# cvYouTian/Dedark-YOLO

Hardware: AMD Instinct MI355X
Metric: training img/s at 640x640 (higher is better)
Workload: dtype bf16

## Files before the change

dedark_yolo_amd/_C.py:

```python
import ctypes as C
import os

_HERE = os.path.dirname(os.path.abspath(__file__))
LIB_PATH = os.path.join(os.environ.get("DY_LIB_DIR") or os.path.join(_HERE, "lib"), "libdedark_yolo.so")

DY_F32, DY_BF16, DY_F16 = 0, 1, 2
ACT_NONE, ACT_SILU, ACT_LEAKY = 0, 1, 2
OPT_RULES = dict(Adam=0, Adamax=1, NAdam=2, RAdam=3, RMSProp=4)
STATS_REPLICAS = 64
BN_BWD_REPLICAS = 8

vp, i32, i64, f32, f64 = C.c_void_p, C.c_int, C.c_int64, C.c_float, C.c_double


class ConvDesc(C.Structure):
    _fields_ = [("src", vp), ("src_ld", i64), ("N", i32), ("Hs", i32), ("Ws", i32), ("Cs", i32), ("w", vp), ("dst", vp),
                ("dst_ld", i64), ("Hd", i32), ("Wd", i32), ("Cd", i32), ("KH", i32), ("KW", i32), ("stride", i32),
                ("pad", i32), ("dil", i32), ("scale", vp), ("shift", vp), ("act", i32), ("stats", vp), ("accumulate", i32),
                ("dtype", i32), ("dst_row_stride", i64), ("dst_img_stride", i64), ("KHf", i32), ("KWf", i32), ("kh0", i32),
                ("kh_step", i32), ("kw0", i32), ("kw_step", i32), ("dst_valid_channels", i32), ("dst_planar", vp),
                ("add_src", vp), ("add_src_ld", i64)]


class PackItem(C.Structure):
    _fields_ = [("w", vp), ("packed", vp), ("Cout", i32), ("Cout_pad", i32), ("Cin", i32), ("Cin_pad", i32), ("KH", i32),
                ("KW", i32), ("transposed", i32), ("dtype", i32), ("first_block", i64)]


class DetMaps(C.Structure):
    _fields_ = [("map", vp * 3), ("map_ld", i64 * 3), ("h", i32 * 3), ("w", i32 * 3), ("stride", f32 * 3), ("B", i32),
                ("nc", i32), ("n_levels", i32), ("dtype", i32)]


class DetMaps4(DetMaps):
    _fields_ = [("map3", vp), ("map_ld3", i64), ("h3", i32), ("w3", i32), ("stride3", f32)]


class AugSample(C.Structure):
    _fields_ = [("src", vp * 4), ("sh", i32 * 4), ("sw", i32 * 4), ("pitch", i64 * 4), ("rect", (i32 * 6) * 4), ("n_src", i32),
                ("canvas_h", i32), ("canvas_w", i32), ("hsv", i32), ("flipud", i32), ("fliplr", i32), ("minv", C.c_double * 6),
                ("lut", (C.c_uint8 * 256) * 3)]


class AugMixSample(C.Structure):
    _fields_ = [("a", AugSample), ("b", AugSample), ("r", C.c_double), ("r1", C.c_double), ("mix", i32)]


class SegDesc(C.Structure):
    _fields_ = [("mc", vp), ("mc_ld", i64), ("proto", vp), ("proto_ld", i64), ("B", i32), ("A", i32), ("nm", i32), ("mh", i32),
                ("mw", i32), ("target_gt_idx", vp), ("fg_mask", vp), ("target_box", vp), ("masks", vp), ("mask_dtype", i32),
                ("mask_h", i32), ("mask_w", i32), ("overlap", i32), ("gt_rows", vp), ("n_max", i32), ("img_h", f32), ("img_w", f32),
                ("pos", vp), ("npos", vp), ("dtype", i32)]


BIAS_GRAD_CHUNKS = 2048
LN_MAX_C = 2048
LN_MAX_PARTS = 512

POSE_MAX_LEVELS = 4


class PoseDesc(C.Structure):
    _fields_ = [("kpt", vp * POSE_MAX_LEVELS), ("kpt_ld", i64 * POSE_MAX_LEVELS), ("h", i32 * POSE_MAX_LEVELS), ("w", i32 * POSE_MAX_LEVELS),
                ("stride", f32 * POSE_MAX_LEVELS), ("n_levels", i32), ("B", i32), ("A", i32), ("K", i32), ("ndim", i32), ("dtype", i32),
                ("target_gt_idx", vp), ("fg_mask", vp), ("target_box", vp), ("keypoints", vp), ("n_targets", i32), ("gt_rows", vp),
                ("n_max", i32), ("img_h", f32), ("img_w", f32), ("sigma", vp), ("pos", vp), ("npos", vp)]


_SIGS = {
    "dy_version": [],
    "dy_frontend_init": [],
    "dy_conv2d_fwd": [C.POINTER(ConvDesc), vp],
    "dy_conv2d_dgrad": [C.POINTER(ConvDesc), vp],
    "dy_conv2d_wgrad": [vp, i64, i32, i32, i32, i32, vp, i64, i32, i32, i32, i32, i32, i32, i32, i32, i32, i32, vp, i64, vp,
                        i32, vp],
    "dy_conv2d_wgrad_forked": [vp, vp, i64, i32, i32, i32, i32, vp, i64, i32, i32, i32, i32, i32, i32, i32, i32, i32, i32, vp, i64,
                               vp, i32, vp],
    "dy_conv2d_bn_act_fwd": [C.POINTER(ConvDesc), i64, vp, vp, vp, vp, f32, f32, vp, i32, vp, i64, vp, i64, vp],
    "dy_bn_act_bwd": [vp, i64, vp, i64, vp, vp, i32, vp, vp, i64, vp, vp, i64, i32, i32, vp],
# ... 182 lines not shown
```

dedark_yolo_amd/csrc/conv.hip:

```cpp
#include <stdlib.h>
#include "dy_host.h"
#include "conv_epilogue.h"
#include "../../include/dedark_yolo.h"
#include "conv_route.h"

namespace {

constexpr int ROWB = 144;
constexpr int NTHREADS = 256;

struct ConvP {
  const char* src;
  long src_ld;
  int N, Hs, Ws, Cs;
  const char* w;
  char* dst;
  long dst_ld;
  int Hd, Wd, Cd;
  int KH, KW, stride, pad, dil;
  const float* scale;
  const float* shift;
  int act;
  double* stats;
  int accumulate;
// ... 637 lines not shown

template <typename T>
__global__ void pack_weight_kernel(const float* __restrict__ w, T* __restrict__ out, int Cout, int Cout_pad, int Cin,
                                   int Cin_pad, int KH, int KW, int transposed) {
  long total = (long)Cout_pad * KH * KW * Cin_pad;
  for (long i = blockIdx.x * (long)blockDim.x + threadIdx.x; i < total; i += (long)gridDim.x * blockDim.x) {
    int co, kh, kw, ci;
    long r = i;
    if (!transposed) {
      ci = (int)(r % Cin_pad); r /= Cin_pad;
      kw = (int)(r % KW); r /= KW;
      kh = (int)(r % KH); r /= KH;
      co = (int)r;
    } else {
      co = (int)(r % Cout_pad); r /= Cout_pad;
      kw = (int)(r % KW); r /= KW;
      kh = (int)(r % KH); r /= KH;
      ci = (int)r;
    }
    float v = (ci < Cin && co < Cout) ? w[(((long)co * Cin + ci) * KH + kh) * KW + kw] : 0.f;
    DT<T>::st(out + i, v);
  }
}

constexpr int PACK_TILE = 32, PACK_TAPS = 9;

__device__ inline void pack_store(const dy_pack_item& it, long o, float v) {
  if (it.dtype == DY_F32) ((float*)it.packed)[o] = v;
  else if (it.dtype == DY_F16) ((f16_t*)it.packed)[o] = (f16_t)v;
  else ((bf16_t*)it.packed)[o] = f32_to_bf16(v);
}

template <int TC>
__device__ inline void pack_chunk(const dy_pack_item& it, float (&tile)[PACK_TILE][PACK_TILE * PACK_TAPS + 1], int co0, int ci0, int T,
                                  int t0, int tc_rt) {
  const int tc = TC ? TC : tc_rt;
  const int tid = threadIdx.x;
  const int run = PACK_TILE * tc;
  {
    const int r = tid >> 3, co = co0 + r;
    const bool row_ok = co < it.Cout;
    const float* src = it.w + ((long)co * it.Cin + ci0) * T + t0;
    for (int k = tid & 7; k < run; k += 8) {
      const int cl = k / tc, t = k - cl * tc;
      const int ci = ci0 + cl;
      float v = 0.f;
      if (row_ok && ci < it.Cin) v = src[(long)cl * T + t];
      tile[r][cl * PACK_TAPS + t] = v;
    }
  }
  __syncthreads();
  const int VE = it.dtype == DY_F32 ? 4 : 8, GP = PACK_TILE / VE;
  const int n_vec = PACK_TILE * GP * tc;
  for (int i = tid; i < n_vec; i += 256) {
    const int g = i % GP, q = i / GP;
    const int a = q / tc, t = q - a * tc;
    float v[8];
    long o;
    bool ok;
    if (!it.transposed) {
      const int co = co0 + a, ci = ci0 + g * VE;
#pragma unroll
      for (int e = 0; e < 8; ++e) v[e] = e < VE ? tile[a][(g * VE + e) * PACK_TAPS + t] : 0.f;
      ok = co < it.Cout_pad && ci < it.Cin_pad;
      o = ((long)co * T + t0 + t) * it.Cin_pad + ci;
    } else {
      const int ci = ci0 + a, co = co0 + g * VE;
#pragma unroll
      for (int e = 0; e < 8; ++e) v[e] = e < VE ? tile[g * VE + e][a * PACK_TAPS + t] : 0.f;
      ok = co < it.Cout_pad && ci < it.Cin_pad;
      o = ((long)ci * T + t0 + t) * it.Cout_pad + co;
    }
    if (!ok) continue;
    if (it.dtype == DY_F32) stvec<float>((float*)it.packed + o, v);
    else if (it.dtype == DY_F16) stvec<f16_t>((f16_t*)it.packed + o, v);
    else stvec<bf16_t>((bf16_t*)it.packed + o, v);
  }
  __syncthreads();
}

__global__ __launch_bounds__(256) void pack_multi_kernel(const dy_pack_item* __restrict__ items, int n_items) {
  __shared__ float tile[PACK_TILE][PACK_TILE * PACK_TAPS + 1];
  __shared__ long fb[1024];
  const long b = blockIdx.x;
  const bool cached = n_items <= 1024;
  if (cached) {
    for (int i = threadIdx.x; i < n_items; i += 256) fb[i] = items[i].first_block;
    __syncthreads();
  }
  int lo = 0, hi = n_items - 1;
  while (lo < hi) {
    const int mid = (lo + hi + 1) >> 1;
    if ((cached ? fb[mid] : items[mid].first_block) <= b) lo = mid; else hi = mid - 1;
  }
  const dy_pack_item it = items[lo];
  const int tiles_ci = (it.Cin_pad + PACK_TILE - 1) / PACK_TILE;
  const int tb = (int)(b - it.first_block);
  const int co0 = (tb / tiles_ci) * PACK_TILE, ci0 = (tb % tiles_ci) * PACK_TILE;
  const int T = it.KH * it.KW;
  if (T == 9) pack_chunk<9>(it, tile, co0, ci0, 9, 0, 9);
  else if (T == 1) pack_chunk<1>(it, tile, co0, ci0, 1, 0, 1);
  else
    for (int t0 = 0; t0 < T; t0 += PACK_TAPS) pack_chunk<0>(it, tile, co0, ci0, T, t0, T - t0 < PACK_TAPS ? T - t0 : PACK_TAPS);
}

template <typename T, int MODE>
int launch_conv(const dy_conv_desc* d, hipStream_t st, const dy_conv_desc* classes, int ncls) {
  ConvP p;
  dy_route::fill_parity_classes(p, classes, ncls);
  dy_route::fill_gather(p, d);
  constexpr int BM = 128;
  const int tiles_m = dy_cdiv(p.M, BM);
  auto blocks = [&](int bn) {
    p.tiles_n = dy_cdiv(d->Cd, bn);
    p.nblk = tiles_m * p.tiles_n;
    if (p.ncls > 1) p.nblk = dy_route::number_parity_blocks(p, BM, dy_route::CLS_SEQUENTIAL);
  };
  dy_note_kernel(d->Cd <= 32 ? "conv_igemm_kernel<BN=32>" : (d->Cd <= 64 ? "conv_igemm_kernel<BN=64>" : "conv_igemm_kernel<BN=128>"));
  if (d->Cd <= 32) {
    blocks(32);
    conv_igemm_kernel<T, BM, 32, 4, 1, MODE><<<p.nblk, NTHREADS, 0, st>>>(p);
  } else if (d->Cd <= 64) {
    blocks(64);
    conv_igemm_kernel<T, BM, 64, 2, 2, MODE><<<p.nblk, NTHREADS, 0, st>>>(p);
  } else {
    blocks(128);
    conv_igemm_kernel<T, BM, 128, 2, 2, MODE><<<p.nblk, NTHREADS, 0, st>>>(p);
  }
  DY_LAUNCH_CHECK();
// ... 326 lines not shown
```

dedark_yolo_amd/csrc/conv_epilogue.h:

```cpp
#pragma once
#include "dy_common.h"

namespace dy_epi {

template <int BM>
constexpr int pitch() { return BM * 2 + 8; }

typedef __attribute__((ext_vector_type(4))) short s16x4;
typedef __attribute__((address_space(3))) s16x4* lds_s16x4_ptr;

template <int BM, int BN>
constexpr int image_bytes() { return BN * pitch<BM>(); }

template <typename T16 = bf16_t>
__device__ inline uint32_t pack2(float a, float b) {
  if constexpr (__is_same(T16, bf16_t)) return pack_bf16x2(a, b);
  else return (uint32_t)cvt16<T16>(a) | ((uint32_t)cvt16<T16>(b) << 16);
}

template <int BM, int BN, int NW, typename T16, typename OffFn>
__device__ inline void store_image(const char* smem, int lane, int wave, long m0, int n0, long M, int Cd, int accumulate, T16* dst,
                                   OffFn off) {
  constexpr int PT = pitch<BM>();
  constexpr int UP = BM / 16, UC = BN / 32;
  const int g = lane >> 4, li = lane & 15, tq = li >> 2, tp = li & 3;
  static_assert(UP % NW == 0, "pixel tiles per wave");
#pragma unroll 2
  for (int u = 0; u < (UP / NW) * UC; ++u) {
    const int pt = wave + NW * (u / UC), ct = u % UC;
    const int cb = ct * 32 + 8 * g;
    const char* base = smem + (cb + tq) * PT + (pt * 16 + 4 * tp) * 2;
    const s16x4 lo = __builtin_amdgcn_ds_read_tr16_b64_v4i16((lds_s16x4_ptr)(base));
    const s16x4 hi = __builtin_amdgcn_ds_read_tr16_b64_v4i16((lds_s16x4_ptr)(base + 4 * PT));
    const long m = m0 + pt * 16 + li;
    const int n = n0 + cb;
    if (m < M && n < Cd) {
      u32x4 v;
      v[0] = (uint32_t)(uint16_t)lo[0] | ((uint32_t)(uint16_t)lo[1] << 16);
      v[1] = (uint32_t)(uint16_t)lo[2] | ((uint32_t)(uint16_t)lo[3] << 16);
      v[2] = (uint32_t)(uint16_t)hi[0] | ((uint32_t)(uint16_t)hi[1] << 16);
      v[3] = (uint32_t)(uint16_t)hi[2] | ((uint32_t)(uint16_t)hi[3] << 16);
      T16* o = dst + off(m) + n;
      if (n + 8 <= Cd) {
        if (accumulate) {
          float x[8], y[8];
          ldvec<T16>(o, x);
          ldvec<T16>(reinterpret_cast<const T16*>(&v), y);
#pragma unroll
          for (int e = 0; e < 8; ++e) x[e] += y[e];
          stvec<T16>(o, x);
        } else {
          *reinterpret_cast<u32x4*>(o) = v;
        }
      } else {
        const T16* e = reinterpret_cast<const T16*>(&v);
        for (int q = 0; q < 8 && n + q < Cd; ++q) {
          if (accumulate) DT<T16>::st(o + q, DT<T16>::ld(o + q) + DT<T16>::ld(e + q));
          else o[q] = e[q];
        }
      }
    }
  }
}

template <int BN>
constexpr int row_pitch() { return BN * 2 + 8; }

template <int BM, int BN>
constexpr int row_image_bytes() { return BM * row_pitch<BN>(); }

template <int BM, int BN, int NW, typename T16, typename OffFn, int RG = 64>
__device__ inline void store_rows(const char* smem, int lane, int wave, long m0, int n0, long M, int Cd, int accumulate, T16* dst, OffFn off,
                                  const T16* __restrict__ add = nullptr, long add_ld = 0) {
  constexpr int PT = row_pitch<BN>();
  constexpr int LPP = BN >= 128 ? 16 : BN / 8;
  constexpr int PPI = 64 / LPP;
  constexpr int ITERS = BM / PPI / NW;
  constexpr int HALVES = BN >= 128 ? BN / 128 : 1;
  const int pl = lane / LPP, chunk = lane % LPP;
  const bool nt = accumulate & 2;
  accumulate &= 1;
#pragma unroll 2
  for (int u = 0; u < ITERS; ++u) {
    const int px = PPI * (wave + NW * u) + pl;
    if (RG < 64 && (px & 63) >= RG) continue;
    const long m = RG < 64 ? m0 + (px >> 6) * RG + (px & 63) : m0 + px;
#pragma unroll
    for (int h = 0; h < HALVES; ++h) {
      const int c = 128 * h + 8 * chunk;
      const uint2 lo = *reinterpret_cast<const uint2*>(smem + px * PT + c * 2);
      const uint2 hi = *reinterpret_cast<const uint2*>(smem + px * PT + c * 2 + 8);
      const int n = n0 + c;
      if (m < M && n < Cd) {
        u32x4 v = {lo.x, lo.y, hi.x, hi.y};
        T16* o = dst + off(m) + n;
        if (n + 8 <= Cd) {
          if (accumulate || add) {
            float x[8], y[8];
            ldvec<T16>(reinterpret_cast<const T16*>(&v), y);
            if (accumulate) {
              ldvec<T16>(o, x);
#pragma unroll
              for (int e = 0; e < 8; ++e) y[e] += x[e];
            }
            if (add) {
              ldvec<T16>(add + m * add_ld + n, x);
#pragma unroll
              for (int e = 0; e < 8; ++e) y[e] += x[e];
            }
            if (nt) {
              u32x4 w;
              stvec<T16>(reinterpret_cast<T16*>(&w), y);
              asm volatile("global_store_dwordx4 %0, %1, off nt" ::"v"(o), "v"(w) : "memory");
            } else {
              stvec<T16>(o, y);
            }
          } else if (nt) {
            asm volatile("global_store_dwordx4 %0, %1, off nt" ::"v"(o), "v"(v) : "memory");
          } else {
            *reinterpret_cast<u32x4*>(o) = v;
          }
        } else {
          const T16* e = reinterpret_cast<const T16*>(&v);
          for (int q = 0; q < 8 && n + q < Cd; ++q) {
            float t = DT<T16>::ld(e + q);
            if (accumulate) t += DT<T16>::ld(o + q);
            if (add) t += DT<T16>::ld(add + m * add_ld + n + q);
            DT<T16>::st(o + q, t);
          }
        }
      }
    }
  }
}
// ... 48 lines not shown
```

dedark_yolo_amd/csrc/conv_v4.hip:

```cpp
#include <stdlib.h>
#include <type_traits>
#include "dy_host.h"
#include "conv_epilogue.h"
#include "../../include/dedark_yolo.h"
#include "conv_route.h"

namespace v4 {

constexpr int BM = 256, BN = 256, BK = 64;
constexpr int HALF = 128 * 128;
constexpr int OFF_A0 = 0, OFF_A1 = HALF, OFF_B0 = 2 * HALF, OFF_B1 = 3 * HALF, BUF = 4 * HALF;
constexpr unsigned B_ROW_OOB = 0x40000000u;

typedef __attribute__((address_space(3))) void* lds_ptr_t;
typedef __attribute__((ext_vector_type(8))) __bf16 bf16x8;

struct P {
  const char* src;
  const char* w;
  char* dst;
  unsigned src_bytes, w_bytes;
  long src_ld, dst_ld, dst_row, dst_img;
  int Hs, Ws, Cs, Hd, Wd, Cd;
  int stride;
// ... 248 lines not shown
    for (int i = 0; i < 4; ++i)
      for (int j = 0; j < 3; ++j) o[3 * i + j] = t_sum[i][j];
  }
  if (!(ABL & 8) && wr == 0) __builtin_amdgcn_s_barrier();
  asm volatile("s_waitcnt vmcnt(0)" ::: "memory");
  __builtin_amdgcn_s_barrier();

  constexpr int PT = dy_epi::row_pitch<BN>();
  const int cl = lane & 15, g = lane >> 4;
  const bool plain = !p.scale && !p.shift && p.act == DY_ACT_NONE;
#pragma unroll
  for (int bh = 0; bh < 2; ++bh)
#pragma unroll
    for (int j = 0; j < 2; ++j) {
      const int c0 = 128 * bh + 32 * wc + 16 * j + 4 * g;
      if (plain) {
#pragma unroll
        for (int ah = 0; ah < 2; ++ah)
#pragma unroll
          for (int i = 0; i < RB; ++i) {
            const int px = 128 * ah + 64 * wr + 16 * i + cl;
            uint2 w2 = {dy_epi::pack2<T>(acc[ah][bh][i][j][0], acc[ah][bh][i][j][1]), dy_epi::pack2<T>(acc[ah][bh][i][j][2], acc[ah][bh][i][j][3])};
            *reinterpret_cast<uint2*>(smem + px * PT + c0 * 2) = w2;
          }
      } else {
        float sc[4], sf[4];
#pragma unroll
        for (int e = 0; e < 4; ++e) {
          const int n = n0 + c0 + e;
          const bool nok = n < p.Cd;
          sc[e] = (nok && p.scale) ? p.scale[n] : 1.f;
          sf[e] = (nok && p.shift) ? p.shift[n] : 0.f;
        }
#pragma unroll
        for (int ah = 0; ah < 2; ++ah)
#pragma unroll
          for (int i = 0; i < RB; ++i) {
            const int px = 128 * ah + 64 * wr + 16 * i + cl;
            float v[4];
#pragma unroll
            for (int e = 0; e < 4; ++e) {
              float u = acc[ah][bh][i][j][e] * sc[e] + sf[e];
              if (p.act == DY_ACT_SILU) u = u * dy_sigmoid(u);
              else if (p.act == DY_ACT_LEAKY) u = u > 0.f ? u : 0.1f * u;
              v[e] = u;
            }
            uint2 w2 = {dy_epi::pack2<T>(v[0], v[1]), dy_epi::pack2<T>(v[2], v[3])};
            *reinterpret_cast<uint2*>(smem + px * PT + c0 * 2) = w2;
          }
      }
    }
  __syncthreads();
  auto off_fn = [&](long m) { return dst_offset(p, m); };
  if (!(ABL & 64))
    dy_epi::store_rows<BM, BN, 8, T, decltype(off_fn), RG>(smem, lane, wave, m0, n0, p.M, p.Cd, p.accumulate, reinterpret_cast<T*>(p.dst), off_fn,
                                                           reinterpret_cast<const T*>(p.add_src), p.add_src_ld);
  if (p.stats && !(ABL & 512)) {
    __syncthreads();
    float* red = reinterpret_cast<float*>(smem);
#pragma unroll
    for (int bh = 0; bh < 2; ++bh)
#pragma unroll
      for (int j = 0; j < 2; ++j)
#pragma unroll
        for (int e = 0; e < 4; ++e) {
          float s1 = 0.f, s2 = 0.f;
#pragma unroll
          for (int ah = 0; ah < 2; ++ah)
#pragma unroll
            for (int i = 0; i < RB; ++i) {
              const float a = acc[ah][bh][i][j][e];
              s1 += a;
              s2 += a * a;
            }
          s1 = row16_sum(s1);
          s2 = row16_sum(s2);
          if (cl == 0) {
            const int col = 128 * bh + 32 * wc + 16 * j + 4 * g + e;
            red[(wr * BN + col) * 2] = s1;
            red[(wr * BN + col) * 2 + 1] = s2;
          }
        }
    __syncthreads();
    if (tid < BN) {
      const int n = n0 + tid;
      if (n < p.Cd) {
        const float s1 = red[tid * 2] + red[(BN + tid) * 2];
        const float s2 = red[tid * 2 + 1] + red[(BN + tid) * 2 + 1];
        double* st = p.stats + (long)(tile_m % DY_STATS_REPLICAS) * 2 * p.Cd;
        atomic_add_f64(st + n, (double)s1);
        atomic_add_f64(st + p.Cd + n, (double)s2);
      }
    }
  }
}

template <int ABL, typename T = bf16_t>
__global__ __launch_bounds__(512) void conv_kernel(const P p) {
  extern __shared__ __attribute__((aligned(16))) char smem[];
  if (p.ncls > 1) {
    const int x = blockIdx.x & 7, i = (int)blockIdx.x >> 3;
    int c = 0;
#pragma unroll
    for (int k = 1; k < 4; ++k)
      if (k < p.ncls && i >= p.cls[k].blk0) c = k;
    const DyParityCls& k = p.cls[c];
// ... 141 lines not shown
```

dedark_yolo_amd/csrc/conv_v5.hip:

```cpp
#include <stdlib.h>
#include <type_traits>
#include "dy_host.h"
#include "conv_epilogue.h"
#include "../../include/dedark_yolo.h"
#include "conv_route.h"

namespace v5 {

constexpr int BM = 256, BK = 32;
constexpr int A_BYTES = BM * 64, NSTAGE = 3;
constexpr unsigned B_ROW_OOB = 0x40000000u;

typedef __attribute__((address_space(3))) void* lds_ptr_t;
typedef __attribute__((ext_vector_type(8))) __bf16 bf16x8;

__device__ unsigned long long g_stamps[16];

__device__ inline void stamp(int ablate, int nblk, int i) {
  if ((ablate & 32) && threadIdx.x == 0 && (blockIdx.x == 0 || (int)blockIdx.x == (nblk / 8) * 7)) {
    unsigned long long t;
    asm volatile("s_memtime %0\n\ts_waitcnt lgkmcnt(0)" : "=s"(t)::"memory");
    g_stamps[(blockIdx.x == 0 ? 0 : 8) + i] = t;
  }
}
// ... 23 lines not shown
  long add_src_ld;
  int ablate;
  int ncls;
  DyParityCls cls[4];
};

using dy_route::xcd_remap;
using dy_route::dst_offset;

template <int BN, typename T, int MB>
__device__ __forceinline__ void epilogue(const P& p, f32x4 (&acc)[MB][4], char* smem, int tid, int lane, int wave, int wm, int wn, long m0,
                                         int n0, int tile_m) {
  constexpr int WN = BN / 64, WM = 4 / WN;
  constexpr int PT = dy_epi::row_pitch<BN>();
  const int cl = lane & 15, g = lane >> 4;
  const bool plain = !p.scale && !p.shift && p.act == DY_ACT_NONE;
#pragma unroll
  for (int j = 0; j < 4; ++j) {
    const int c0 = 64 * wn + 16 * j + 4 * g;
    if (plain) {
#pragma unroll
      for (int i = 0; i < MB; ++i) {
        const int px = 16 * MB * wm + 16 * i + cl;
        uint2 w2 = {dy_epi::pack2<T>(acc[i][j][0], acc[i][j][1]), dy_epi::pack2<T>(acc[i][j][2], acc[i][j][3])};
        *reinterpret_cast<uint2*>(smem + px * PT + c0 * 2) = w2;
      }
    } else {
      float sc[4], sf[4];
#pragma unroll
      for (int e = 0; e < 4; ++e) {
        const int n = n0 + c0 + e;
        const bool nok = n < p.Cd;
        sc[e] = (nok && p.scale) ? p.scale[n] : 1.f;
        sf[e] = (nok && p.shift) ? p.shift[n] : 0.f;
      }
#pragma unroll
      for (int i = 0; i < MB; ++i) {
        const int px = 16 * MB * wm + 16 * i + cl;
        float v[4];
#pragma unroll
        for (int e = 0; e < 4; ++e) {
          float u = acc[i][j][e] * sc[e] + sf[e];
          if (p.act == DY_ACT_SILU) u = u * dy_sigmoid(u);
          else if (p.act == DY_ACT_LEAKY) u = u > 0.f ? u : 0.1f * u;
          v[e] = u;
        }
        uint2 w2 = {dy_epi::pack2<T>(v[0], v[1]), dy_epi::pack2<T>(v[2], v[3])};
        *reinterpret_cast<uint2*>(smem + px * PT + c0 * 2) = w2;
      }
    }
  }
  __syncthreads();
  stamp(DY_ABLATE_OF(p), p.nblk, 3);
  dy_epi::store_rows<BM, BN, 4>(smem, lane, wave, m0, n0, p.M, p.Cd, p.accumulate, reinterpret_cast<T*>(p.dst),
                                [&](long m) { return dst_offset(p, m); }, reinterpret_cast<const T*>(p.add_src), p.add_src_ld);
  stamp(DY_ABLATE_OF(p), p.nblk, 4);
  if (p.stats) {
    __syncthreads();
    float* red = reinterpret_cast<float*>(smem);
#pragma unroll
    for (int j = 0; j < 4; ++j)
#pragma unroll
      for (int e = 0; e < 4; ++e) {
        float s1 = 0.f, s2 = 0.f;
#pragma unroll
        for (int i = 0; i < MB; ++i) {
          const float a = acc[i][j][e];
          s1 += a;
          s2 += a * a;
        }
        s1 = row16_sum(s1);
        s2 = row16_sum(s2);
        if (cl == 0) {
          const int col = 64 * wn + 16 * j + 4 * g + e;
          red[(wm * BN + col) * 2] = s1;
          red[(wm * BN + col) * 2 + 1] = s2;
        }
      }
    __syncthreads();
    if (tid < BN) {
      const int n = n0 + tid;
      if (n < p.Cd) {
        float s1 = 0.f, s2 = 0.f;
#pragma unroll
        for (int w = 0; w < WM; ++w) {
          s1 += red[(w * BN + tid) * 2];
          s2 += red[(w * BN + tid) * 2 + 1];
        }
        double* st = p.stats + (long)(tile_m % DY_STATS_REPLICAS) * 2 * p.Cd;
        atomic_add_f64(st + n, (double)s1);
        atomic_add_f64(st + p.Cd + n, (double)s2);
      }
    }
  }
}

template <int BN, typename T = bf16_t, bool SLIM = false>
__global__ __launch_bounds__(256, SLIM ? 4 : 2) void conv_kernel(const P pk) {
  constexpr int WN = BN / 64, WM = 4 / WN, MB = BM / WM / 16, NB = 4, STAGE = A_BYTES + BN * 64, B_LD = BN / 64;
  extern __shared__ __attribute__((aligned(16))) char smem[];
  const int tid = threadIdx.x, lane = tid & 63;
  const int wave = __builtin_amdgcn_readfirstlane(tid >> 6);
  const int wm = wave / WN, wn = wave % WN;
  P p = pk;
  int bid;
  if (pk.ncls > 1) {
    const int x = blockIdx.x & 7, i = (int)blockIdx.x >> 3;
    int c = 0;
// ... 504 lines not shown
```

dedark_yolo_amd/ops.py:

```python
import ctypes as C
import math
import os
import weakref

import torch

from . import _C
from ._C import ACT_LEAKY, ACT_NONE, ACT_SILU, ConvDesc, DetMaps, DetMaps4, call

_compute_dtype = torch.float32
_pack_generation = 0
_weights_epoch = 0


def set_compute_dtype(dt):
    global _compute_dtype
    if dt not in (torch.float32, torch.bfloat16, torch.float16):
        raise ValueError(f"dedark_yolo_amd: unsupported compute dtype {dt}")
    _compute_dtype = dt


def get_compute_dtype():
    return _compute_dtype

# ... 183 lines not shown

arena = _Arena()


def _w32(weight):
    w = weight.detach()
    if w.dtype != torch.float32 or not w.is_contiguous():
        w = w.float().contiguous()
    return w


def _pack(weight, cout_pad, cin_pad, transposed, dtype):
    key = (cout_pad, cin_pad, transposed, dtype)
    cache = weight.__dict__.setdefault("_dy_pack", {})
    hit = cache.get(key)
    tag = (_weights_epoch, weight._version)
    if hit is not None and hit[0] == tag:
        return hit[1]
    Co, Ci, KH, KW = weight.shape
    if hit is None:
        global _pack_generation
        _pack_generation += 1
    out = hit[1] if hit is not None else torch.empty(cout_pad * KH * KW * cin_pad, dtype=dtype, device=weight.device)
    w32 = _w32(weight)
    call("dy_pack_weight", ptr(w32), ptr(out), Co, cout_pad, Ci, cin_pad, KH, KW, 1 if transposed else 0, dt_id(dtype), stream())
    cache[key] = (tag, out)
    return out


_extra_pack_views = []


def register_pack_view(t):
    _extra_pack_views.append(weakref.ref(t))


def weight_view(p, shape, r0=None, r1=None):
    cache = p.__dict__.setdefault("_dy_views", {})
    key = (tuple(shape), r0, r1)
    hit = cache.get(key)
    at = p.data_ptr()
    if hit is None or hit[0] != at:
        w = p.detach()
        hit = cache[key] = (at, (w if r0 is None else w[r0:r1]).view(shape))
        register_pack_view(hit[1])
    return hit[1]


class PackPlan:

    def __init__(self):
        self.sig = None
        self.table = None
        self.n_blocks = 0
        self._ent_key = None
        self._ent = []
        self._ent_sig = ()

    def _collect(self, model):
        ent = []
        _extra_pack_views[:] = [r for r in _extra_pack_views if r() is not None]
        for w in list(model.parameters()) + [r() for r in _extra_pack_views]:
            cache = w.__dict__.get("_dy_pack")
            if not cache or w.dtype != torch.float32 or not w.is_contiguous() or w.dim() != 4:
                continue
            for key, (tag, out) in cache.items():
                ent.append((w, key, out))
        return ent

    def repack(self, model):
        key = (id(model), _pack_generation)
        if key != self._ent_key:
            self._ent = self._collect(model)
            self._ent_sig = tuple((w.data_ptr(), out.data_ptr(), k) for w, k, out in self._ent)
            self._ent_key = key
        ent = self._ent
        if not ent:
            return
        sig = self._ent_sig
        if any(w.data_ptr() != sg[0] for (w, _, _), sg in zip(ent[:4], sig[:4])):
            self._ent_key = None
            return self.repack(model)
        if sig != self.sig:
            items = (_C.PackItem * len(ent))()
            blk = 0
            lib = _C.lib()
            for it, (w, (cout_pad, cin_pad, transposed, dtype), out) in zip(items, ent):
                Co, Ci, KH, KW = w.shape
                it.w, it.packed = w.data_ptr(), out.data_ptr()
                it.Cout, it.Cout_pad, it.Cin, it.Cin_pad, it.KH, it.KW = Co, cout_pad, Ci, cin_pad, KH, KW
                it.transposed, it.dtype, it.first_block = int(transposed), dt_id(dtype), blk
                blk += lib.dy_pack_item_blocks(cout_pad, cin_pad, KH, KW)
            raw = torch.frombuffer(bytearray(bytes(items)), dtype=torch.uint8)
            self.table = raw.to(ent[0][0].device)
            self.n_blocks, self.sig = blk, sig
        call("dy_pack_weights_multi", ptr(self.table), len(ent), self.n_blocks, stream())
        for w, key, out in ent:
            w.__dict__["_dy_pack"][key] = ((_weights_epoch, w._version), out)


def _padded_vec(v, n):
    if v is None:
        return None
    v = v.detach()
    if v.numel() == n and v.dtype == torch.float32:
        return v
    out = torch.zeros(n, dtype=torch.float32, device=v.device)
    out[:v.numel()] = v
    return out


def bn_fold(bn, cout_pad):
    tag = (_weights_epoch, bn.weight._version, bn.bias._version, bn.running_mean._version, bn.running_var._version,
           bn.weight.data_ptr(), bn.running_mean.data_ptr(), cout_pad)
    hit = bn.__dict__.get("_dy_fold")
    if hit is not None and hit[0] == tag:
        return hit[1]
    aff = hit[1] if (hit is not None and hit[1].shape[1] == cout_pad and hit[1].device == bn.weight.device) else \
        torch.empty((2, cout_pad), dtype=torch.float32, device=bn.weight.device)
    call("dy_bn_fold_eval_valid", ptr(bn.weight), ptr(bn.bias), ptr(bn.running_mean), ptr(bn.running_var), float(bn.eps),
         ptr(aff[0]), ptr(aff[1]), cout_pad, bn.weight.numel(), stream())
    bn.__dict__["_dy_fold"] = (tag, aff)
    return aff


def bn_fold_is_current(bn):
    hit = bn.__dict__.get("_dy_fold")
    return hit is not None and hit[0][:7] == (_weights_epoch, bn.weight._version, bn.bias._version, bn.running_mean._version,
                                               bn.running_var._version, bn.weight.data_ptr(), bn.running_mean.data_ptr())


class ConvCtx:
    __slots__ = ("x", "z", "aff", "weight", "bias", "bn", "act", "k", "stride", "pad", "dil", "cout", "cout_pad", "cin_pad",
                 "has_bn", "y", "owner", "shared")


def _conv_desc(src, w, dst, N, Hs, Ws, Cs, Hd, Wd, Cd, KH, KW, stride, pad, dil, scale, shift, act, stats, accumulate, dtype):
    if dst is not None:
        dptr, dld = dst.data_ptr(), ld_of(dst)
    else:
        dptr, dld = None, Cd
    return ConvDesc(src.data_ptr(), ld_of(src), N, Hs, Ws, Cs, w.data_ptr(), dptr, dld, Hd, Wd, Cd, KH, KW, stride, pad, dil,
                    None if scale is None else scale.data_ptr(), None if shift is None else shift.data_ptr(), act,
                    None if stats is None else stats.data_ptr(), 1 if accumulate else 0, dt_id(dtype))


_bn_pending = {}


# ... 1266 lines not shown
```

include/dedark_yolo.h:

```cpp
#ifndef DEDARK_YOLO_H
#define DEDARK_YOLO_H
#include <stddef.h>
#include <stdint.h>
#ifdef __cplusplus
extern "C" {
#endif

#define DY_F32 0
#define DY_BF16 1
#define DY_F16 2
#define DY_ACT_NONE 0
#define DY_ACT_SILU 1
#define DY_ACT_LEAKY 2
#define DY_STATS_REPLICAS 64
#define DY_BN_BWD_REPLICAS 8

const char* dy_last_error(void);
int dy_version(void);
const char* dy_last_kernel(void);
void dy_clear_last_kernel(void);

typedef struct {
  const void* src;
  int64_t src_ld;
  int N, Hs, Ws, Cs;
  const void* w;
  void* dst;
  int64_t dst_ld;
  int Hd, Wd, Cd;
  int KH, KW, stride, pad, dil;
  const float* scale;
  const float* shift;
  int act;
  double* stats;
  int accumulate;
  int dtype;
  int64_t dst_row_stride;
  int64_t dst_img_stride;
  int KHf, KWf;
  int kh0, kh_step;
  int kw0, kw_step;
  int dst_valid_channels;
  void* dst_planar;
  const void* add_src;
  int64_t add_src_ld;
} dy_conv_desc;

int dy_conv2d_fwd(const dy_conv_desc* d, void* stream);
int dy_conv2d_dgrad(const dy_conv_desc* d, void* stream);
int dy_conv2d_wgrad(const void* x, int64_t x_ld, int N, int Hi, int Wi, int Cin_pad, const void* dz, int64_t dz_ld, int Ho,
                    int Wo, int Cout_pad, int KH, int KW, int stride, int pad, int dil, int Cout, int Cin, float* scratch,
                    int64_t scratch_elems, float* g_oihw, int dtype, void* stream);
int dy_pack_weight(const float* w_oihw, void* packed, int Cout, int Cout_pad, int Cin, int Cin_pad, int KH, int KW,
                   int transposed, int dtype, void* stream);
typedef struct {
  const float* w;
  void* packed;
  int Cout, Cout_pad, Cin, Cin_pad, KH, KW, transposed, dtype;
  int64_t first_block;
} dy_pack_item;
int64_t dy_pack_item_blocks(int Cout_pad, int Cin_pad, int KH, int KW);
int dy_pack_weights_multi(const dy_pack_item* items_dev, int n_items, int64_t n_blocks, void* stream);

int dy_bn_finalize(const double* stats, int64_t count, const float* gamma, const float* beta, float* running_mean,
                   float* running_var, float momentum, float eps, float* scale, float* shift, float* mean, float* invstd,
                   int C, void* stream);
int dy_bn_fold_eval(const float* gamma, const float* beta, const float* running_mean, const float* running_var, float eps,
                    float* scale, float* shift, int C, void* stream);
int dy_bn_finalize_valid(const double* stats, int64_t count, const float* gamma, const float* beta, float* running_mean,
                         float* running_var, float momentum, float eps, float* scale, float* shift, float* mean, float* invstd,
                         int C, int C_valid, void* stream);
int dy_bn_fold_eval_valid(const float* gamma, const float* beta, const float* running_mean, const float* running_var, float eps,
                          float* scale, float* shift, int C, int C_valid, void* stream);
int dy_bn_act_fwd(const void* z, int64_t z_ld, const float* scale, const float* shift, int act, const void* residual,
                  int64_t res_ld, void* y, int64_t y_ld, int64_t pixels, int C, int dtype, void* stream);
int dy_bn_act_bwd_reduce(const void* dy, int64_t dy_ld, const void* z, int64_t z_ld, const float* scale,
                         const float* shift, const float* mean, const float* invstd, int act, int has_bn, double* sums,
                         int64_t pixels, int C, int dtype, void* stream);
int dy_bn_act_bwd_apply(const void* dy, int64_t dy_ld, const void* z, int64_t z_ld, const float* scale, const float* shift,
                        const float* mean, const float* invstd, const float* gamma, int act, int has_bn,
                        const double* sums, void* dz, int64_t dz_ld, float* dgamma, float* dbeta, int64_t pixels, int C,
                        int dtype, void* stream);
int dy_bn_act_bwd_apply_valid(const void* dy, int64_t dy_ld, const void* z, int64_t z_ld, const float* scale, const float* shift,
                              const float* mean, const float* invstd, const float* gamma, int act, int has_bn,
                              const double* sums, void* dz, int64_t dz_ld, float* dgamma, float* dbeta, int64_t pixels, int C,
                              int C_valid, int dtype, void* stream);

int dy_bn2_act_fwd(const void* u, int64_t u_ld, const void* v, int64_t v_ld, const float* scale_u, const float* shift_u,
                   const float* scale_v, const float* shift_v, int act, void* y, int64_t y_ld, int64_t pixels, int C, int dtype,
                   void* stream);
#define DY_BN2_MAX_PARTS 1024
int64_t dy_bn2_act_bwd_workspace(int64_t pixels, int C, int dtype);
int dy_bn2_act_bwd(const void* dy, int64_t dy_ld, const void* u, int64_t u_ld, const void* v, int64_t v_ld, const float* scale_u,
                   const float* shift_u, const float* mean_u, const float* invstd_u, const float* gamma_u, const float* scale_v,
                   const float* shift_v, const float* mean_v, const float* invstd_v, const float* gamma_v, int act, void* du,
                   int64_t du_ld, void* dv, int64_t dv_ld, float* dgamma_u, float* dbeta_u, float* dgamma_v, float* dbeta_v,
                   float* workspace, int64_t workspace_elems, int64_t pixels, int C, int dtype, void* stream);

int dy_maxpool_fwd(const void* x, int64_t x_ld, void* y, int64_t y_ld, uint8_t* argmax, int N, int H, int W, int C, int k,
                   int stride, int pad, int Ho, int Wo, int dtype, void* stream);
int dy_maxpool_bwd(const void* dy, int64_t dy_ld, const uint8_t* argmax, void* dx, int64_t dx_ld, int N, int H, int W, int C,
                   int k, int stride, int pad, int Ho, int Wo, int accumulate, int dtype, void* stream);
int dy_upsample_nearest_fwd(const void* x, int64_t x_ld, void* y, int64_t y_ld, int N, int H, int W, int C, int scale,
                            int dtype, void* stream);
int dy_upsample_nearest_bwd(const void* dy, int64_t dy_ld, void* dx, int64_t dx_ld, int N, int H, int W, int C, int scale,
                            int accumulate, int dtype, void* stream);
int dy_copy2d(const void* src, int64_t src_ld, void* dst, int64_t dst_ld, int64_t pixels, int C, int accumulate, int dtype,
              void* stream);
int dy_cast(const void* src, int src_dtype, void* dst, int dst_dtype, int64_t n, void* stream);

int dy_pconv_pack(const float* w, void* wp, int c3, int transposed, int dtype, void* stream);
int dy_pconv_fwd(const void* x, int64_t x_ld, void* y, int64_t y_ld, const float* w, const void* wp, int N, int H, int W, int C, int c3,
// ... 295 lines not shown
```

Baseline: 1039.

## Pack plain and transposed weights in one pass; buffer-load accumulate epilogue

```diff
diff --git a/dedark_yolo_amd/_C.py b/dedark_yolo_amd/_C.py
--- a/dedark_yolo_amd/_C.py
+++ b/dedark_yolo_amd/_C.py
@@ -24,7 +24,7 @@
 
 class PackItem(C.Structure):
     _fields_ = [("w", vp), ("packed", vp), ("Cout", i32), ("Cout_pad", i32), ("Cin", i32), ("Cin_pad", i32), ("KH", i32),
-                ("KW", i32), ("transposed", i32), ("dtype", i32), ("first_block", i64)]
+                ("KW", i32), ("transposed", i32), ("dtype", i32), ("first_block", i64), ("packed_t", vp)]
 
 
 class DetMaps(C.Structure):
diff --git a/dedark_yolo_amd/csrc/conv.hip b/dedark_yolo_amd/csrc/conv.hip
--- a/dedark_yolo_amd/csrc/conv.hip
+++ b/dedark_yolo_amd/csrc/conv.hip
@@ -713,29 +713,33 @@
   __syncthreads();
   const int VE = it.dtype == DY_F32 ? 4 : 8, GP = PACK_TILE / VE;
   const int n_vec = PACK_TILE * GP * tc;
-  for (int i = tid; i < n_vec; i += 256) {
-    const int g = i % GP, q = i / GP;
-    const int a = q / tc, t = q - a * tc;
-    float v[8];
-    long o;
-    bool ok;
-    if (!it.transposed) {
-      const int co = co0 + a, ci = ci0 + g * VE;
-#pragma unroll
-      for (int e = 0; e < 8; ++e) v[e] = e < VE ? tile[a][(g * VE + e) * PACK_TAPS + t] : 0.f;
-      ok = co < it.Cout_pad && ci < it.Cin_pad;
-      o = ((long)co * T + t0 + t) * it.Cin_pad + ci;
-    } else {
-      const int ci = ci0 + a, co = co0 + g * VE;
-#pragma unroll
-      for (int e = 0; e < 8; ++e) v[e] = e < VE ? tile[g * VE + e][a * PACK_TAPS + t] : 0.f;
-      ok = co < it.Cout_pad && ci < it.Cin_pad;
-      o = ((long)ci * T + t0 + t) * it.Cout_pad + co;
-    }
-    if (!ok) continue;
-    if (it.dtype == DY_F32) stvec<float>((float*)it.packed + o, v);
-    else if (it.dtype == DY_F16) stvec<f16_t>((f16_t*)it.packed + o, v);
-    else stvec<bf16_t>((bf16_t*)it.packed + o, v);
+  for (int lay = 0; lay < (it.packed_t ? 2 : 1); ++lay) {
+    const bool transposed = lay ? !it.transposed : (bool)it.transposed;
+    void* const dst = lay ? it.packed_t : it.packed;
+    for (int i = tid; i < n_vec; i += 256) {
+      const int g = i % GP, q = i / GP;
+      const int a = q / tc, t = q - a * tc;
+      float v[8];
+      long o;
+      bool ok;
+      if (!transposed) {
+        const int co = co0 + a, ci = ci0 + g * VE;
+#pragma unroll
+        for (int e = 0; e < 8; ++e) v[e] = e < VE ? tile[a][(g * VE + e) * PACK_TAPS + t] : 0.f;
+        ok = co < it.Cout_pad && ci < it.Cin_pad;
+        o = ((long)co * T + t0 + t) * it.Cin_pad + ci;
+      } else {
+        const int ci = ci0 + a, co = co0 + g * VE;
+#pragma unroll
+        for (int e = 0; e < 8; ++e) v[e] = e < VE ? tile[g * VE + e][a * PACK_TAPS + t] : 0.f;
+        ok = co < it.Cout_pad && ci < it.Cin_pad;
+        o = ((long)ci * T + t0 + t) * it.Cout_pad + co;
+      }
+      if (!ok) continue;
+      if (it.dtype == DY_F32) stvec<float>((float*)dst + o, v);
+      else if (it.dtype == DY_F16) stvec<f16_t>((f16_t*)dst + o, v);
+      else stvec<bf16_t>((bf16_t*)dst + o, v);
+    }
   }
   __syncthreads();
 }
diff --git a/dedark_yolo_amd/csrc/conv_epilogue.h b/dedark_yolo_amd/csrc/conv_epilogue.h
--- a/dedark_yolo_amd/csrc/conv_epilogue.h
+++ b/dedark_yolo_amd/csrc/conv_epilogue.h
@@ -71,7 +71,7 @@
 
 template <int BM, int BN, int NW, typename T16, typename OffFn, int RG = 64>
 __device__ inline void store_rows(const char* smem, int lane, int wave, long m0, int n0, long M, int Cd, int accumulate, T16* dst, OffFn off,
-                                  const T16* __restrict__ add = nullptr, long add_ld = 0) {
+                                  const T16* __restrict__ add = nullptr, long add_ld = 0, long dense_ld = 0) {
   constexpr int PT = row_pitch<BN>();
   constexpr int LPP = BN >= 128 ? 16 : BN / 8;
   constexpr int PPI = 64 / LPP;
@@ -80,6 +80,65 @@
   const int pl = lane / LPP, chunk = lane % LPP;
   const bool nt = accumulate & 2;
   accumulate &= 1;
+  if (dense_ld && (accumulate || add) && (Cd & 7) == 0 && dense_ld < (1 << 22) && add_ld < (1 << 22)) {
+    constexpr int NB = BN >= 128 ? 8 : 4;
+    static_assert(NB % HALVES == 0 && ITERS % (NB / HALVES) == 0, "whole batches");
+    constexpr int UB = NB / HALVES;
+    constexpr uint32_t NEG0 = 0x80008000u;
+    constexpr uint32_t SKIP = 0x80000000u;
+    const long rows = M - 1 - m0;
+    const auto extent = [&](long ld) {
+      const long bytes = (rows * ld + Cd) * 2;
+      return rows < 0 ? 0 : (int)(bytes < 0x7fffffffL ? bytes : 0x7fffffffL);
+    };
+    const __amdgpu_buffer_rsrc_t rs_d = __builtin_amdgcn_make_buffer_rsrc((void*)(dst + m0 * dense_ld), 0, extent(dense_ld), 0x00020000);
+    const __amdgpu_buffer_rsrc_t rs_a =
+        __builtin_amdgcn_make_buffer_rsrc((void*)(add ? add + m0 * add_ld : dst), 0, add ? extent(add_ld) : 0, 0x00020000);
+    const int ld_d = (int)dense_ld, ld_a = (int)add_ld;
+    for (int u0 = 0; u0 < ITERS; u0 += UB) {
+      u32x4 dv[NB], av[NB];
+      uint32_t od[NB];
+#pragma unroll
+      for (int j = 0; j < UB; ++j) {
+        const int px = PPI * (wave + NW * (u0 + j)) + pl;
+        const int r = RG < 64 ? (px >> 6) * RG + (px & 63) : px;
+        const bool mok = (RG == 64 || (px & 63) < RG) && m0 + r < M;
+#pragma unroll
+        for (int h = 0; h < HALVES; ++h) {
+          const int k = j * HALVES + h;
+          const int n = n0 + 128 * h + 8 * chunk;
+          const bool ok = mok && n + 8 <= Cd;
+          od[k] = ok ? (uint32_t)(r * ld_d + n) * 2u : SKIP;
+          dv[k] = u32x4{NEG0, NEG0, NEG0, NEG0};
+          av[k] = u32x4{NEG0, NEG0, NEG0, NEG0};
+          if (accumulate) dv[k] = __builtin_amdgcn_raw_buffer_load_b128(rs_d, (int)od[k], 0, 0);
+          if (add) av[k] = __builtin_amdgcn_raw_buffer_load_b128(rs_a, (int)(ok ? (uint32_t)(r * ld_a + n) * 2u : SKIP), 0, 0);
+        }
+      }
+#pragma unroll
+      for (int k = 0; k < NB; ++k) {
+        __builtin_amdgcn_sched_barrier(0);
+        const int px = PPI * (wave + NW * (u0 + k / HALVES)) + pl;
+        const int c = 128 * (k % HALVES) + 8 * chunk;
+        const uint2 lo = *reinterpret_cast<const uint2*>(smem + px * PT + c * 2);
+        const uint2 hi = *reinterpret_cast<const uint2*>(smem + px * PT + c * 2 + 8);
+        const u32x4 v = {lo.x, lo.y, hi.x, hi.y};
+        float x[8], y[8];
+        ldvec<T16>(reinterpret_cast<const T16*>(&v), y);
+        ldvec<T16>(reinterpret_cast<const T16*>(&dv[k]), x);
+#pragma unroll
+        for (int e = 0; e < 8; ++e) y[e] += x[e];
+        ldvec<T16>(reinterpret_cast<const T16*>(&av[k]), x);
+#pragma unroll
+        for (int e = 0; e < 8; ++e) y[e] += x[e];
+        u32x4 w;
+        stvec<T16>(reinterpret_cast<T16*>(&w), y);
+        if (nt) __builtin_amdgcn_raw_buffer_store_b128(w, rs_d, (int)od[k], 0, 2);
+        else __builtin_amdgcn_raw_buffer_store_b128(w, rs_d, (int)od[k], 0, 0);
+      }
+    }
+    return;
+  }
 #pragma unroll 2
   for (int u = 0; u < ITERS; ++u) {
     const int px = PPI * (wave + NW * u) + pl;
diff --git a/dedark_yolo_amd/csrc/conv_v4.hip b/dedark_yolo_amd/csrc/conv_v4.hip
--- a/dedark_yolo_amd/csrc/conv_v4.hip
+++ b/dedark_yolo_amd/csrc/conv_v4.hip
@@ -324,6 +324,12 @@
     }
   __syncthreads();
   auto off_fn = [&](long m) { return dst_offset(p, m); };
+  if (!p.stats && p.dst_row == 0 && ((p.accumulate & 1) || p.add_src)) {
+    if (!(ABL & 64))
+      dy_epi::store_rows<BM, BN, 8, T, decltype(off_fn), RG>(smem, lane, wave, m0, n0, p.M, p.Cd, p.accumulate, reinterpret_cast<T*>(p.dst), off_fn,
+                                                             reinterpret_cast<const T*>(p.add_src), p.add_src_ld, p.dst_ld);
+    return;
+  }
   if (!(ABL & 64))
     dy_epi::store_rows<BM, BN, 8, T, decltype(off_fn), RG>(smem, lane, wave, m0, n0, p.M, p.Cd, p.accumulate, reinterpret_cast<T*>(p.dst), off_fn,
                                                            reinterpret_cast<const T*>(p.add_src), p.add_src_ld);
diff --git a/dedark_yolo_amd/csrc/conv_v5.hip b/dedark_yolo_amd/csrc/conv_v5.hip
--- a/dedark_yolo_amd/csrc/conv_v5.hip
+++ b/dedark_yolo_amd/csrc/conv_v5.hip
@@ -99,8 +99,15 @@
   }
   __syncthreads();
   stamp(DY_ABLATE_OF(p), p.nblk, 3);
-  dy_epi::store_rows<BM, BN, 4>(smem, lane, wave, m0, n0, p.M, p.Cd, p.accumulate, reinterpret_cast<T*>(p.dst),
-                                [&](long m) { return dst_offset(p, m); }, reinterpret_cast<const T*>(p.add_src), p.add_src_ld);
+  auto off_fn = [&](long m) { return dst_offset(p, m); };
+  if (!p.stats && p.dst_row == 0 && ((p.accumulate & 1) || p.add_src)) {
+    dy_epi::store_rows<BM, BN, 4>(smem, lane, wave, m0, n0, p.M, p.Cd, p.accumulate, reinterpret_cast<T*>(p.dst), off_fn,
+                                  reinterpret_cast<const T*>(p.add_src), p.add_src_ld, p.dst_ld);
+    stamp(DY_ABLATE_OF(p), p.nblk, 4);
+    return;
+  }
+  dy_epi::store_rows<BM, BN, 4>(smem, lane, wave, m0, n0, p.M, p.Cd, p.accumulate, reinterpret_cast<T*>(p.dst), off_fn,
+                                reinterpret_cast<const T*>(p.add_src), p.add_src_ld);
   stamp(DY_ABLATE_OF(p), p.nblk, 4);
   if (p.stats) {
     __syncthreads();
diff --git a/dedark_yolo_amd/ops.py b/dedark_yolo_amd/ops.py
--- a/dedark_yolo_amd/ops.py
+++ b/dedark_yolo_amd/ops.py
@@ -259,6 +259,7 @@
     def __init__(self):
         self.sig = None
         self.table = None
+        self.n_items = 0
         self.n_blocks = 0
         self._ent_key = None
         self._ent = []
@@ -289,19 +290,27 @@
             self._ent_key = None
             return self.repack(model)
         if sig != self.sig:
-            items = (_C.PackItem * len(ent))()
+            groups = {}
+            for w, (cout_pad, cin_pad, transposed, dtype), out in ent:
+                ve = vec_elems(dtype)
+                if cout_pad % ve or cin_pad % ve or out.data_ptr() % 16:
+                    raise RuntimeError(f"PackPlan: packed extents ({cout_pad}, {cin_pad}) / pointer are no multiples of the {ve}-element vector")
+                groups.setdefault((id(w), cout_pad, cin_pad, dtype), [w, None, None])[1 + int(bool(transposed))] = out
+            items = (_C.PackItem * len(groups))()
             blk = 0
             lib = _C.lib()
-            for it, (w, (cout_pad, cin_pad, transposed, dtype), out) in zip(items, ent):
+            for it, ((_, cout_pad, cin_pad, dtype), (w, plain, transp)) in zip(items, groups.items()):
                 Co, Ci, KH, KW = w.shape
-                it.w, it.packed = w.data_ptr(), out.data_ptr()
+                first = plain if plain is not None else transp
+                it.w, it.packed = w.data_ptr(), first.data_ptr()
+                it.packed_t = transp.data_ptr() if plain is not None and transp is not None else None
                 it.Cout, it.Cout_pad, it.Cin, it.Cin_pad, it.KH, it.KW = Co, cout_pad, Ci, cin_pad, KH, KW
-                it.transposed, it.dtype, it.first_block = int(transposed), dt_id(dtype), blk
+                it.transposed, it.dtype, it.first_block = int(plain is None), dt_id(dtype), blk
                 blk += lib.dy_pack_item_blocks(cout_pad, cin_pad, KH, KW)
             raw = torch.frombuffer(bytearray(bytes(items)), dtype=torch.uint8)
             self.table = raw.to(ent[0][0].device)
-            self.n_blocks, self.sig = blk, sig
-        call("dy_pack_weights_multi", ptr(self.table), len(ent), self.n_blocks, stream())
+            self.n_items, self.n_blocks, self.sig = len(groups), blk, sig
+        call("dy_pack_weights_multi", ptr(self.table), self.n_items, self.n_blocks, stream())
         for w, key, out in ent:
             w.__dict__["_dy_pack"][key] = ((_weights_epoch, w._version), out)
 
diff --git a/include/dedark_yolo.h b/include/dedark_yolo.h
--- a/include/dedark_yolo.h
+++ b/include/dedark_yolo.h
@@ -58,6 +58,7 @@
   void* packed;
   int Cout, Cout_pad, Cin, Cin_pad, KH, KW, transposed, dtype;
   int64_t first_block;
+  void* packed_t;
 } dy_pack_item;
 int64_t dy_pack_item_blocks(int Cout_pad, int Cin_pad, int KH, int KW);
 int dy_pack_weights_multi(const dy_pack_item* items_dev, int n_items, int64_t n_blocks, void* stream);
```

Result: no change. 1049 (median of 6 runs) (+0.9%).
